# nalinbhardwaj/curdleproofs.pie

Measured on AMD Instinct MI355X. Metric: BLS12-381 G1 scalar-muls/sec at MSM size 2^20, higher is better.
Workload: dtype u32

## Files before the change

### curdleproofs_pie_amd/csrc/kernels_reduce.h

```cpp
#pragma once

__global__ void __launch_bounds__(256) k_seg_reduce(const uint32_t* __restrict__ choff, const PointSum* __restrict__ sums,
                                                    const uint8_t* __restrict__ combined,
                                                    PointSum* __restrict__ seg_run, PointSum* __restrict__ seg_tot,
                                                    uint32_t nseg_total, uint32_t m) {
  uint32_t s = blockIdx.x * 256 + threadIdx.x;
  if (s >= nseg_total) return;
  xyzz run = xyzz_identity(), tot = xyzz_identity();
  for (int t = (int)m - 1; t >= 0; --t) {
    uint32_t b = s * m + (uint32_t)t;
    uint32_t c0 = choff[b], c1 = choff[b + 1];
    if (combined[b]) c1 = c0 + 1;
    for (uint32_t k = c0; k < c1; ++k) run = xyzz_add(run, load_sum(sums + k));
    tot = xyzz_add(tot, run);
  }
  store_sum(seg_run + s, run);
  store_sum(seg_tot + s, tot);
}


constexpr uint32_t BT_ELEMS = 2048;
__global__ void __launch_bounds__(256) k_bit_tree(const PointSum* __restrict__ seg_run, const PointSum* __restrict__ seg_tot,
                                                  PointSum* __restrict__ partial, uint32_t J) {
  __shared__ PointSum sh[4];
  const uint32_t item = blockIdx.x, lw = blockIdx.y, S = gridDim.z, z = blockIdx.z;
  const PointSum* src = (item == 0 ? seg_tot : seg_run) + (size_t)lw * J;
  const uint32_t count = (item == 0) ? J : (J >> 1);
  const uint32_t e0 = z * BT_ELEMS, e1 = (e0 + BT_ELEMS < count) ? e0 + BT_ELEMS : count;
  xyzz acc = xyzz_identity();
  const uint32_t b = item - 1;
  for (uint32_t e = e0 + threadIdx.x; e < e1; e += 256) {
    uint32_t j = (item == 0) ? e : ((((e >> b) << 1) | 1u) << b) | (e & ((1u << b) - 1u));
    acc = xyzz_add(acc, load_sum(src + j));
  }
  for (int delta = 32; delta >= 1; delta >>= 1) {
    xyzz o = shfl_down_xyzz(acc, delta);
    if ((threadIdx.x & 63) < (uint32_t)delta) acc = xyzz_add(acc, o);
  }
  if ((threadIdx.x & 63) == 0) store_sum(&sh[threadIdx.x >> 6], acc);
  __syncthreads();
  if (threadIdx.x < 64) {
    acc = (threadIdx.x < 4) ? load_sum(&sh[threadIdx.x]) : xyzz_identity();
    for (int delta = 2; delta >= 1; delta >>= 1) {
      xyzz o = shfl_down_xyzz(acc, delta);
      if (threadIdx.x < (uint32_t)delta) acc = xyzz_add(acc, o);
    }
    if (threadIdx.x == 0) store_sum(partial + ((size_t)lw * gridDim.x + item) * S + z, acc);
  }
}

__global__ void __launch_bounds__(64) k_bit_tree_final(const PointSum* __restrict__ partial, PointWords* __restrict__ out, uint32_t S) {
  const size_t idx = blockIdx.x;
  xyzz acc = (threadIdx.x < S) ? load_sum(partial + idx * S + threadIdx.x) : xyzz_identity();
  for (int delta = 32; delta >= 1; delta >>= 1) {
    if ((uint32_t)delta >= S) continue;
    xyzz o = shfl_down_xyzz(acc, delta);
    if (threadIdx.x < (uint32_t)delta) acc = xyzz_add(acc, o);
  }
  if (threadIdx.x == 0) {
    xyzz_words o;
    xyzz_export(acc, o);
    PointWords* dst = out + idx;
    for (int cidx = 0; cidx < 4; ++cidx) for (int k = 0; k < 12; ++k) dst->w[cidx][k] = o.w[cidx][k];
    dst->inf = o.inf;
  }
}

__device__ __forceinline__ xyzz bucket_sum(const uint32_t* __restrict__ choff, const PointSum* __restrict__ sums,
                                           const uint8_t* __restrict__ combined, uint32_t b) {
  uint32_t c0 = choff[b], c1 = choff[b + 1];
  if (combined[b]) c1 = c0 + 1;
  xyzz acc = xyzz_identity();
  for (uint32_t k = c0; k < c1; ++k) acc = xyzz_add(acc, load_sum(sums + k));
  return acc;
}

__device__ __forceinline__ xyzz group_tree(xyzz acc, uint32_t lanes, uint32_t part, uint32_t base, int use_quad) {
  uint32_t delta = lanes >> 1;
  for (; delta >= 1 && (!use_quad || delta * 4u > lanes); delta >>= 1) {
    xyzz o = shfl_down_xyzz(acc, (int)delta);
    if (part < delta) acc = xyzz_add(acc, o);
  }
  uint32_t stride = 1;
  const uint32_t q = part & 3u, quad = part >> 2;
  for (; delta >= 1; delta >>= 1) {
    const uint32_t v = quad < delta ? quad : 0u;
    const xyzz a = shfl_xyzz(acc, (int)(base + v * stride));
    const xyzz b = shfl_xyzz(acc, (int)(base + (v + delta) * stride));
    acc = quad_add(a, b, q);
    stride = 4;
  }
  return acc;
}

__global__ void __launch_bounds__(256, 2) k_rowcol(const uint32_t* __restrict__ choff, const PointSum* __restrict__ sums,
                                                const uint8_t* __restrict__ combined, PointSum* __restrict__ rowsum,
                                                PointSum* __restrict__ colsum, uint32_t nlw, uint32_t hb, uint32_t lb,
                                                uint32_t nrow_blocks, int use_quad) {
  const uint32_t R = 1u << hb, Cn = 1u << lb;
  const uint32_t lane = threadIdx.x & 63u;
  if (blockIdx.x < nrow_blocks) {
    const uint32_t lpr = Cn < 32u ? Cn : 32u, serial = Cn / lpr;
    const uint32_t gr = blockIdx.x * (256u / lpr) + threadIdx.x / lpr;
    const uint32_t part = threadIdx.x % lpr;
    const bool live = gr < nlw * R;
    xyzz acc = xyzz_identity();
    if (live)
      for (uint32_t t = 0; t < serial; ++t) acc = xyzz_add(acc, bucket_sum(choff, sums, combined, gr * Cn + part * serial + t));
    acc = group_tree(acc, lpr, part, lane - part, use_quad && lpr >= 4u);
    if (live && part == 0) store_sum(rowsum + gr, acc);
  } else {
    const uint32_t lpc = R < 16u ? R : 16u, serial = R / lpc;
    const uint32_t gc = (blockIdx.x - nrow_blocks) * (256u / lpc) + threadIdx.x / lpc;
    const uint32_t part = threadIdx.x % lpc;
    const bool live = gc < nlw * Cn;
    const uint32_t lw = gc / Cn, l = gc % Cn;
    xyzz acc = xyzz_identity();
    if (live)
      for (uint32_t t = 0; t < serial; ++t) acc = xyzz_add(acc, bucket_sum(choff, sums, combined, (lw * R + part * serial + t) * Cn + l));
    acc = group_tree(acc, lpc, part, lane - part, use_quad && lpc >= 4u);
    if (live && part == 0) store_sum(colsum + gc, acc);
  }
}

__global__ void __launch_bounds__(256, 2) k_bucket_fold_quad(const uint32_t* __restrict__ choff, PointSum* __restrict__ sums,
                                                             uint8_t* __restrict__ combined, uint32_t nb_total,
                                                             const uint32_t* __restrict__ any_multi) {
  if (*any_multi == 0u) return;
  const uint32_t t = blockIdx.x * 256 + threadIdx.x, b = t >> 2, q = t & 3u;
  if (b >= nb_total) return;
  const uint32_t c0 = choff[b], c1 = choff[b + 1];
  if (c1 - c0 < 2u || c1 - c0 >= HEAVY_MIN_CHUNKS) return;
  xyzz acc = load_sum(sums + c0);
#pragma unroll 1
  for (uint32_t k = c0 + 1; k < c1; ++k) acc = quad_add(acc, load_sum(sums + k), q);
  if (q == 0) { store_sum(sums + c0, acc); combined[b] = 1; }
}

__global__ void __launch_bounds__(256, 2) k_rowcol_quad(const uint32_t* __restrict__ choff, const PointSum* __restrict__ sums,
                                                        PointSum* __restrict__ rowsum, PointSum* __restrict__ colsum,
                                                        uint32_t nlw, uint32_t hb, uint32_t lb, uint32_t lgq) {
  const uint32_t R = 1u << hb, Cn = 1u << lb, G = 1u << lgq, per_wave = 16u >> lgq;
  const uint32_t wave = blockIdx.x * 4u + (threadIdx.x >> 6), lane = threadIdx.x & 63u, q = lane & 3u, quad = lane >> 2;
  const uint32_t gw = wave * per_wave + (quad >> lgq), p = quad & (G - 1u);
  const uint32_t nrows = nlw * R, ncols = nlw * Cn;
  if (wave * per_wave >= nrows + ncols) return;
  const bool live_row = gw < nrows + ncols;
  const bool is_row = gw < nrows;
  uint32_t first = 0, stride = 1u;
  const uint32_t len = is_row ? Cn : R;
  if (live_row) {
    if (is_row) { first = gw * Cn; stride = 1u; }
    else { const uint32_t gc = gw - nrows, lw = gc / Cn, l = gc % Cn; first = lw * R * Cn + l; stride = Cn; }
  }
  const uint32_t nser = ((R > Cn ? R : Cn) + G - 1u) >> lgq;
  xyzz acc = xyzz_identity();
#pragma unroll 1
  for (uint32_t step = 0; step < nser + lgq; ++step) {
    xyzz o;
    bool go;
    if (step < nser) {
      const uint32_t i = p + G * step;
      const uint32_t b = first + (i < len ? i : 0u) * stride;
      const uint32_t c0 = choff[b];
      go = live_row && i < len && choff[b + 1] > c0;
      o = load_sum(sums + c0);
    } else {
      const uint32_t dq = (G >> 1) >> (step - nser);
      o = shfl_down_xyzz(acc, (int)(4u * dq));
      go = p < dq;
    }
    if (go) acc = quad_add(acc, o, q);
  }
  if (live_row && p == 0u && q == 0u) store_sum(is_row ? rowsum + gw : colsum + (gw - nrows), acc);
}

__global__ void __launch_bounds__(256, 2) k_rowcol_quad_row(const uint32_t* __restrict__ choff, const PointSum* __restrict__ sums,
                                                            const uint8_t* __restrict__ combined,
                                                            PointSum* __restrict__ rowsum, PointSum* __restrict__ colsum,
                                                            uint32_t nlw, uint32_t hb, uint32_t lb) {
  __shared__ PointSum part[4 * 16];
  const uint32_t R = 1u << hb, Cn = 1u << lb;
  const uint32_t wib = threadIdx.x >> 6, gw = blockIdx.x * 4u + wib, lane = threadIdx.x & 63u, q = lane & 3u, p = lane >> 2;
  const uint32_t nrows = nlw * R, ncols = nlw * Cn;
  if (gw >= nrows + ncols) return;
  const bool is_row = gw < nrows;
  uint32_t first, stride;
  const uint32_t len = is_row ? Cn : R;
  if (is_row) { first = gw * Cn; stride = 1u; }
  else { const uint32_t gc = gw - nrows, lw = gc / Cn, l = gc % Cn; first = lw * R * Cn + l; stride = Cn; }
  xyzz acc = xyzz_identity();
  uint32_t i = p, c0 = 0, nch = 0, kk = 0;
  bool fresh = true;
#pragma unroll 1
  for (;;) {
    if (fresh) {
      if (i >= len) break;
      const uint32_t b = first + i * stride;
      c0 = choff[b];
      nch = choff[b + 1] - c0;
      if (nch > 1u && combined[b]) nch = 1u;
      kk = 0; i += 16u; fresh = false;
    }
    if (kk < nch) { acc = quad_add(acc, load_sum(sums + c0 + kk), q); ++kk; }
    if (kk >= nch) fresh = true;
  }
  if (q == 0u) store_sum(&part[wib * 16u + p], acc);
  __builtin_amdgcn_wave_barrier();
  __builtin_amdgcn_s_waitcnt(0xc07f);
  const RowK k = row_constants();
  xyzz_row racc = row_load_sum(&part[wib * 16u], k.lane16);
  const uint32_t np = len < 16u ? len : 16u;
#pragma unroll 1
  for (uint32_t j = 1; j < np; ++j) racc = row_add(racc, row_load_sum(&part[wib * 16u + j], k.lane16), k);
  row_store_sum(is_row ? rowsum + gw : colsum + (gw - nrows), racc, k.lane16);
}

__global__ void __launch_bounds__(256) k_small_tree(const PointSum* __restrict__ rowsum, const PointSum* __restrict__ colsum,
                                                    PointWords* __restrict__ out, uint32_t hb, uint32_t lb) {
  __shared__ PointSum sh[4];
  const uint32_t item = blockIdx.x, lw = blockIdx.y;
  const bool on_rows = item <= hb;
  const uint32_t J = on_rows ? (1u << hb) : (1u << lb);
  const PointSum* src = on_rows ? rowsum + (size_t)lw * J : colsum + (size_t)lw * J;
  const uint32_t bit = on_rows ? item - 1u : item - 1u - hb;
  xyzz acc = xyzz_identity();
  if (threadIdx.x < J && (item == 0 || ((threadIdx.x >> bit) & 1u))) acc = load_sum(src + threadIdx.x);
  for (int delta = 32; delta >= 1; delta >>= 1) {
    xyzz o = shfl_down_xyzz(acc, delta);
    if ((threadIdx.x & 63) < (uint32_t)delta) acc = xyzz_add(acc, o);
  }
  if ((threadIdx.x & 63) == 0) store_sum(&sh[threadIdx.x >> 6], acc);
  __syncthreads();
  if (threadIdx.x < 64) {
    acc = (threadIdx.x < 4) ? load_sum(&sh[threadIdx.x]) : xyzz_identity();
    for (int delta = 2; delta >= 1; delta >>= 1) {
      xyzz o = shfl_down_xyzz(acc, delta);
      if (threadIdx.x < (uint32_t)delta) acc = xyzz_add(acc, o);
    }
    if (threadIdx.x == 0) {
      xyzz_words o;
      xyzz_export(acc, o);
      PointWords* dst = out + (size_t)lw * gridDim.x + item;
      for (int cidx = 0; cidx < 4; ++cidx) for (int k = 0; k < 12; ++k) dst->w[cidx][k] = o.w[cidx][k];
      dst->inf = o.inf;
    }
  }
}


__global__ void __launch_bounds__(64) k_export_sums(const PointSum* __restrict__ src, PointWords* __restrict__ out, uint32_t n) {
  const uint32_t i = blockIdx.x * 64 + threadIdx.x;
  if (i >= n) return;
  xyzz_words o;
  xyzz_export(load_sum(src + i), o);
  PointWords* dst = out + i;
  for (int cidx = 0; cidx < 4; ++cidx) for (int k = 0; k < 12; ++k) dst->w[cidx][k] = o.w[cidx][k];
  dst->inf = o.inf;
}

__global__ void __launch_bounds__(1024) k_export_host(const uint4* __restrict__ src, uint4* __restrict__ dst_host, uint32_t nvec,
                                                      uint32_t* __restrict__ flag_host, uint32_t seq) {
  for (uint32_t i = threadIdx.x; i < nvec; i += 1024) dst_host[i] = src[i];
  __threadfence_system();
  __syncthreads();
  if (threadIdx.x == 0) {
    __hip_atomic_store(flag_host, seq, __ATOMIC_RELEASE, __HIP_MEMORY_SCOPE_SYSTEM);
  }
}


__global__ void __launch_bounds__(512) k_small_tree_quad(const PointSum* __restrict__ rowsum, const PointSum* __restrict__ colsum,
                                                         PointWords* __restrict__ out, uint32_t hb, uint32_t lb) {
  __shared__ PointSum sh[8];
  const uint32_t item = blockIdx.x, lw = blockIdx.y;
  const uint32_t q = threadIdx.x & 3u, Q = threadIdx.x >> 2, lane = threadIdx.x & 63u, wave = threadIdx.x >> 6;
  const uint32_t NQ = blockDim.x >> 2, NW = blockDim.x >> 6;
  const bool on_rows = item <= hb;
  const uint32_t J = on_rows ? (1u << hb) : (1u << lb);
  const PointSum* src = on_rows ? rowsum + (size_t)lw * J : colsum + (size_t)lw * J;
  const uint32_t bit = on_rows ? item - 1u : item - 1u - hb;
  xyzz acc = xyzz_identity();
  for (uint32_t e = Q; e < J; e += NQ)
    if (item == 0 || ((e >> bit) & 1u)) acc = quad_add(acc, load_sum(src + e), q);
  for (uint32_t dq = 8; dq >= 1; dq >>= 1) {
    xyzz o = shfl_down_xyzz(acc, (int)(4u * dq));
    if ((lane >> 2) < dq) acc = quad_add(acc, o, q);
  }
  if (NW > 1) {
    if (lane == 0) store_sum(&sh[wave], acc);
    __syncthreads();
    if (wave == 0) {
      acc = (Q < NW) ? load_sum(&sh[Q]) : xyzz_identity();
      for (uint32_t dq = NW >> 1; dq >= 1; dq >>= 1) {
        xyzz o = shfl_down_xyzz(acc, (int)(4u * dq));
        if (Q < dq) acc = quad_add(acc, o, q);
      }
    }
  }
  if (threadIdx.x == 0) {
    xyzz_words o;
    xyzz_export(acc, o);
    PointWords* dst = out + (size_t)lw * gridDim.x + item;
    for (int cidx = 0; cidx < 4; ++cidx) for (int k = 0; k < 12; ++k) dst->w[cidx][k] = o.w[cidx][k];
    dst->inf = o.inf;
  }
}

__global__ void __launch_bounds__(64) k_msm_horner_quad(const PointSum* __restrict__ group_sum, PointWords* __restrict__ out,
                                                        uint32_t M, uint32_t nwin, uint32_t c) {
  const uint32_t t = blockIdx.x * 64 + threadIdx.x, j = t >> 2, q = t & 3u;
  if (j >= M) return;
  xyzz acc = xyzz_identity();
  for (int w = (int)nwin - 1; w >= 0; --w) {
    for (uint32_t k = 0; k < c; ++k) acc = quad_dbl(acc, q);
    acc = quad_add(acc, load_sum(group_sum + (size_t)j * nwin + w), q);
  }
  if (q == 0) {
    xyzz_words o;
    xyzz_export(acc, o);
    PointWords* dst = out + j;
    for (int cidx = 0; cidx < 4; ++cidx) for (int k = 0; k < 12; ++k) dst->w[cidx][k] = o.w[cidx][k];
    dst->inf = o.inf;
  }
}
```

Baseline: 365.7 million.

## Stage bucket-sum loads into LDS with async prefetch in rowcol kernel

Rewrites k_rowcol so the row and column paths share one loop. It prefetches each bucket's first partial sum into LDS with global_load_lds, double-buffered against the xyzz_add of the previous bucket. Multi-chunk buckets are deferred to a wave-uniform walk phase, and the shuffle tree is merged into the same single loop so divergent branches no longer serialize the expensive point adds. The aim is to hide global load latency and cut divergence, at the cost of 60KB of LDS per block, which may limit occupancy, and of more complex waitcnt-based synchronization.

```diff
diff --git a/curdleproofs_pie_amd/csrc/kernels_reduce.h b/curdleproofs_pie_amd/csrc/kernels_reduce.h
--- a/curdleproofs_pie_amd/csrc/kernels_reduce.h
+++ b/curdleproofs_pie_amd/csrc/kernels_reduce.h
@@ -66,31 +66,25 @@
   }
 }
 
-__device__ __forceinline__ xyzz bucket_sum(const uint32_t* __restrict__ choff, const PointSum* __restrict__ sums,
-                                           const uint8_t* __restrict__ combined, uint32_t b) {
-  uint32_t c0 = choff[b], c1 = choff[b + 1];
-  if (combined[b]) c1 = c0 + 1;
-  xyzz acc = xyzz_identity();
-  for (uint32_t k = c0; k < c1; ++k) acc = xyzz_add(acc, load_sum(sums + k));
-  return acc;
-}
-
-__device__ __forceinline__ xyzz group_tree(xyzz acc, uint32_t lanes, uint32_t part, uint32_t base, int use_quad) {
-  uint32_t delta = lanes >> 1;
-  for (; delta >= 1 && (!use_quad || delta * 4u > lanes); delta >>= 1) {
-    xyzz o = shfl_down_xyzz(acc, (int)delta);
-    if (part < delta) acc = xyzz_add(acc, o);
-  }
-  uint32_t stride = 1;
-  const uint32_t q = part & 3u, quad = part >> 2;
-  for (; delta >= 1; delta >>= 1) {
-    const uint32_t v = quad < delta ? quad : 0u;
-    const xyzz a = shfl_xyzz(acc, (int)(base + v * stride));
-    const xyzz b = shfl_xyzz(acc, (int)(base + (v + delta) * stride));
-    acc = quad_add(a, b, q);
-    stride = 4;
-  }
-  return acc;
+constexpr int SUM_PIECES = 15;
+
+__device__ __forceinline__ void stage_sum(const PointSum* src, uint4 (*stage)[64]) {
+  const char* g = reinterpret_cast<const char*>(src);
+#pragma unroll
+  for (int j = 0; j < SUM_PIECES; ++j)
+    __builtin_amdgcn_global_load_lds((const __attribute__((address_space(1))) void*)(g + 16 * j),
+                                     (__attribute__((address_space(3))) void*)&stage[j][0], 16, 0, 0);
+}
+
+__device__ __forceinline__ xyzz staged_sum(const uint4 (*stage)[64], uint32_t lane) {
+  uint32_t w[4 * SUM_PIECES];
+#pragma unroll
+  for (int i = 0; i < SUM_PIECES; ++i) { const uint4 v = stage[i][lane]; w[4 * i] = v.x; w[4 * i + 1] = v.y; w[4 * i + 2] = v.z; w[4 * i + 3] = v.w; }
+  xyzz a;
+#pragma unroll
+  for (int i = 0; i < NL; ++i) { a.X.l[i] = w[i]; a.Y.l[i] = w[NL + i]; a.ZZ.l[i] = w[2 * NL + i]; a.ZZZ.l[i] = w[3 * NL + i]; }
+  a.inf = w[4 * NL];
+  return a;
 }
 
 __global__ void __launch_bounds__(256, 2) k_rowcol(const uint32_t* __restrict__ choff, const PointSum* __restrict__ sums,
@@ -99,28 +93,78 @@
                                                 uint32_t nrow_blocks, int use_quad) {
   const uint32_t R = 1u << hb, Cn = 1u << lb;
   const uint32_t lane = threadIdx.x & 63u;
-  if (blockIdx.x < nrow_blocks) {
-    const uint32_t lpr = Cn < 32u ? Cn : 32u, serial = Cn / lpr;
-    const uint32_t gr = blockIdx.x * (256u / lpr) + threadIdx.x / lpr;
-    const uint32_t part = threadIdx.x % lpr;
-    const bool live = gr < nlw * R;
-    xyzz acc = xyzz_identity();
-    if (live)
-      for (uint32_t t = 0; t < serial; ++t) acc = xyzz_add(acc, bucket_sum(choff, sums, combined, gr * Cn + part * serial + t));
-    acc = group_tree(acc, lpr, part, lane - part, use_quad && lpr >= 4u);
-    if (live && part == 0) store_sum(rowsum + gr, acc);
-  } else {
-    const uint32_t lpc = R < 16u ? R : 16u, serial = R / lpc;
-    const uint32_t gc = (blockIdx.x - nrow_blocks) * (256u / lpc) + threadIdx.x / lpc;
-    const uint32_t part = threadIdx.x % lpc;
-    const bool live = gc < nlw * Cn;
-    const uint32_t lw = gc / Cn, l = gc % Cn;
-    xyzz acc = xyzz_identity();
-    if (live)
-      for (uint32_t t = 0; t < serial; ++t) acc = xyzz_add(acc, bucket_sum(choff, sums, combined, (lw * R + part * serial + t) * Cn + l));
-    acc = group_tree(acc, lpc, part, lane - part, use_quad && lpc >= 4u);
-    if (live && part == 0) store_sum(colsum + gc, acc);
-  }
+  const bool rows = blockIdx.x < nrow_blocks;
+  const uint32_t len = rows ? Cn : R, cap = rows ? 32u : 16u;
+  const uint32_t lpg = len < cap ? len : cap, serial = len / lpg;
+  const uint32_t g = (rows ? blockIdx.x : blockIdx.x - nrow_blocks) * (256u / lpg) + threadIdx.x / lpg;
+  const uint32_t part = threadIdx.x % lpg;
+  const bool live = g < nlw * (rows ? R : Cn);
+  uint32_t b0 = 0, bs = 1u;
+  if (live) {
+    if (rows) b0 = g * Cn + part * serial;
+    else { b0 = (g / Cn * R + part * serial) * Cn + g % Cn; bs = Cn; }
+  }
+  const bool quad_levels = use_quad && lpg >= 4u;
+  __shared__ uint4 stage_all[4][SUM_PIECES][64];
+  uint4 (*stage)[64] = stage_all[threadIdx.x >> 6];
+  uint32_t c0 = choff[b0], nch = choff[b0 + 1] - c0;
+  bool left = false;
+  if (nch > 1u) { if (combined[b0]) nch = 1u; else left = true; }
+  stage_sum(sums + (nch ? c0 : 0u), stage);
+  uint32_t bn = b0 + (serial > 1u ? bs : 0u);
+  uint32_t c0n = choff[bn], c1n = choff[bn + 1];
+  uint32_t wt = 0, wk = 0, wkend = 0;
+  bool walk = false;
+  uint32_t delta = lpg >> 1;
+  xyzz acc = xyzz_identity();
+#pragma unroll 1
+  for (uint32_t step = 0;; ++step) {
+    xyzz o;
+    bool go;
+    if (step < serial) {
+      __builtin_amdgcn_s_waitcnt(0x0f70);
+      o = staged_sum(stage, lane);
+      go = live && nch != 0u;
+      if (step + 1u < serial) {
+        c0 = c0n; nch = c1n - c0n;
+        if (nch > 1u) { if (combined[bn]) nch = 1u; else left = true; }
+        __builtin_amdgcn_s_waitcnt(0xc07f);
+        stage_sum(sums + (nch ? c0 : 0u), stage);
+        bn = b0 + (step + 2u < serial ? step + 2u : step + 1u) * bs;
+        c0n = choff[bn]; c1n = choff[bn + 1];
+      } else {
+        left = left && live;
+        walk = __ballot(left) != 0ull;
+        if (!left) wt = serial;
+      }
+    } else if (walk) {
+      go = wk < wkend;
+      if (go) { o = load_sum(sums + wk); ++wk; }
+      else if (wt < serial) {
+        const uint32_t b = b0 + wt * bs, k0 = choff[b], k1 = choff[b + 1];
+        if (k1 - k0 > 1u && !combined[b]) { wk = k0 + 1u; wkend = k1; }
+        ++wt;
+      }
+      walk = __ballot(wk < wkend || wt < serial) != 0ull;
+    } else {
+      if (delta < 1u || (quad_levels && delta * 4u <= lpg)) break;
+      o = shfl_down_xyzz(acc, (int)delta);
+      go = part < delta;
+      delta >>= 1;
+    }
+    if (go) acc = xyzz_add(acc, o);
+  }
+  const uint32_t base = lane - part, q = part & 3u, quad = part >> 2;
+  uint32_t stride = 1;
+#pragma unroll 1
+  for (; delta >= 1u; delta >>= 1) {
+    const uint32_t v = quad < delta ? quad : 0u;
+    const xyzz a = shfl_xyzz(acc, (int)(base + v * stride));
+    const xyzz b = shfl_xyzz(acc, (int)(base + (v + delta) * stride));
+    acc = quad_add(a, b, q);
+    stride = 4;
+  }
+  if (live && part == 0) store_sum((rows ? rowsum : colsum) + g, acc);
 }
 
 __global__ void __launch_bounds__(256, 2) k_bucket_fold_quad(const uint32_t* __restrict__ choff, PointSum* __restrict__ sums,
```

Measured after the change: 362.3 million. Within noise of the previous version (-0.9%).
